# xcompact3d/x3d2

Hardware: AMD Instinct MI355X
Metric: DoF*steps/s (whole node), TGV 512^3 per GPU, full fractional step (higher is better)
Workload: dtype f64; 1 GPU; TGV 512x512x512 all-periodic, Re=1600, dt=1e-3, RK3 (3 substeps/step), compact6/classic schemes, rocFFT Poisson (configs[2]); per_gpu=512^3, driver=fused, parallelism=domain decomposition 1x1x1, decomposition=yslabs, decomposition_requested=auto, poisson_z_first=228

## Files before the change

### x3d2_amd/csrc/fft512.hip

```cpp
#include "fft_util.h"

#include "fft512_core.h"
#include "spectral000.h"

struct Spec000 {
    const real_t *waves;
    SpecAB t;
    int nx, ny, nz;
    const real_t *rwT;
};

template <int MODE, int NP, bool ZH = false>
__global__ void __launch_bounds__(64 * NP, 16 / NP)
    k_fft512(real2_t *c, const real2_t *__restrict__ twg, long stride_axis, long stride_other, int nxs, Spec000 sp,
             real2_t *xbuf, int ys, int ysc)
{
    extern __shared__ real2_t tile[];
    real2_t *__restrict__ tws = tile + NP * FP;
    if (threadIdx.x < 256) tws[threadIdx.x] = twg[threadIdx.x];
    const int tid = threadIdx.x, l = tid & 63, w = __builtin_amdgcn_readfirstlane(tid >> 6);
    const int i0 = blockIdx.x * NP, m = tid & (NP - 1), r = tid / NP;
    const long base = (long)blockIdx.y * stride_other + i0;
    const bool valid = i0 + m < nxs;
    auto xaddr = [&](int t) {
        const int ch = t / ys, tt = t - ch * ys, pt = tt / ysc, t3 = tt - pt * ysc;
        return ((((long)ch * (ys / ysc) + pt) * gridDim.y + blockIdx.y) * ysc + t3) * nxs + i0 + m;
    };
    real_t rw8[8];
    if (MODE == 2 && valid && !sp.rwT) {
#pragma unroll
        for (int it = 0; it < 8; it++) {
            const real_t wv = sp.waves[((size_t)(it * 64 + r) * sp.ny + blockIdx.y) * nxs + i0 + m];
            rw8[it] = wv < 1.e-16 ? 0.0 : -1.0 / wv;
        }
    }
#pragma unroll
    for (int it = 0; it < 8; it++) {
        const int z = it * 64 + r;
        const real2_t *__restrict__ src = (MODE == 1 && xbuf) ? xbuf + xaddr(z) : c + base + (long)z * stride_axis + m;
        tile[m * FP + z] = valid ? *src : make_real2(0.0, 0.0);
    }
    __syncthreads();
    real2_t *__restrict__ pen = tile + w * FP;
    real2_t a[8];
#pragma unroll
    for (int k = 0; k < 8; k++) a[k] = pen[l + 64 * k];
    if (MODE == 1) fft512_wave<1>(a, pen, tws, l);
    else fft512_wave<-1>(a, pen, tws, l);
    if (MODE == 2 && sp.rwT) {
        const int i = i0 + w, j = blockIdx.y;
        if (i < nxs) {
            const real_t a_o = ZH ? sp.t.az[j] : sp.t.ay[j], b_o = ZH ? sp.t.bz[j] : sp.t.by[j];
            const bool f_o = ZH ? false : (j + 1) > sp.ny / 2 + 1;
            const real_t axi = sp.t.ax[i], bxi = sp.t.bx[i];
            const bool fx = ZH && (i + 1) > sp.nx / 2 + 1;
            const real_t *__restrict__ a_ax = ZH ? sp.t.ay : sp.t.az, *__restrict__ b_ax = ZH ? sp.t.by : sp.t.bz;
            const int n_ax = ZH ? sp.ny : sp.nz;
            const real_t rn = 1.0 / sp.nx / sp.ny / sp.nz;
            const real_t *__restrict__ rwp = sp.rwT + ((size_t)j * nxs + i) * 512;
#pragma unroll
            for (int kk = 0; kk < 8; kk++) {
                const int k = l + 64 * kk;
                real_t div_r = a[kk].x * rn, div_c = a[kk].y * rn;
                const real_t a_k = a_ax[k], b_k = b_ax[k];
                const bool f_k = (k + 1) > n_ax / 2 + 1;
                const Spec000Mode md = ZH ? Spec000Mode{a_o, b_o, a_k, b_k, axi, bxi, f_o, f_k, fx}
                                         : Spec000Mode{a_k, b_k, a_o, b_o, axi, bxi, f_k, f_o, fx};
                spec000_forward(div_r, div_c, md);
                const real_t rw = rwp[k];
                div_r = div_r * rw; div_c = div_c * rw;
                spec000_backward(div_r, div_c, md);
                a[kk] = make_real2(div_r, div_c);
            }
        }
        fft512_wave<1>(a, pen, tws, l);
    } else if (MODE == 2) {
#pragma unroll
        for (int k = 0; k < 8; k++) pen[l + 64 * k] = a[k];
        __syncthreads();
        const int j = blockIdx.y, i = i0 + m;
        if (valid) {
            const real_t ayj = sp.t.ay[j], byj = sp.t.by[j], axi = sp.t.ax[i], bxi = sp.t.bx[i];
            const real_t rn = 1.0 / sp.nx / sp.ny / sp.nz;
            const bool fy = (j + 1) > sp.ny / 2 + 1;
#pragma unroll
            for (int it = 0; it < 8; it++) {
                const int k = it * 64 + r;
                real2_t v = tile[m * FP + k];
                real_t div_r = v.x * rn, div_c = v.y * rn;
                const Spec000Mode md{sp.t.az[k], sp.t.bz[k], ayj, byj, axi, bxi, (k + 1) > sp.nz / 2 + 1, fy, false};
                spec000_forward(div_r, div_c, md);
                const real_t rw = rw8[it];
                div_r = div_r * rw; div_c = div_c * rw;
                spec000_backward(div_r, div_c, md);
                tile[m * FP + k] = make_real2(div_r, div_c);
            }
        }
        __syncthreads();
#pragma unroll
        for (int k = 0; k < 8; k++) a[k] = pen[l + 64 * k];
        __syncthreads();
        fft512_wave<1>(a, pen, tws, l);
    }
#pragma unroll
    for (int k = 0; k < 8; k++) pen[l + 64 * k] = a[k];
    __syncthreads();
    if (valid) {
#pragma unroll
        for (int it = 0; it < 8; it++) {
            const int z = it * 64 + r;
            real2_t *__restrict__ dstp = (MODE == 0 && xbuf) ? xbuf + xaddr(z) : c + base + (long)z * stride_axis + m;
            *dstp = tile[m * FP + z];
        }
    }
}

template <int S, int N>
__device__ __forceinline__ void dft_small(real2_t (&v)[8])
{
    if constexpr (N == 8) fft8<S>(v);
    else if constexpr (N == 4) {
        const real2_t c0 = cadd(v[0], v[2]), c1 = cadd(v[1], v[3]), c2 = csub(v[0], v[2]), d = csub(v[1], v[3]);
        const real2_t c3 = make_real2(-S * d.y, S * d.x);
        v[0] = cadd(c0, c1); v[2] = csub(c0, c1); v[1] = cadd(c2, c3); v[3] = csub(c2, c3);
    } else if constexpr (N == 2) {
        const real2_t t0 = cadd(v[0], v[1]), t1 = csub(v[0], v[1]);
        v[0] = t0; v[1] = t1;
    }
}

struct SpecSlab {
    const real_t *waves;
    SpecAB t;
    int nx, ny, nz, nxs, yoff;
    int xoff;
// ... 112 lines not shown
template <int S, int N>
__global__ void __launch_bounds__(256) k_radix_peers(real2_t *R, long W)
{
    const long w = (long)blockIdx.x * 256 + threadIdx.x;
    const int zl = blockIdx.y;
    if (w >= W) return;
    real2_t v[8];
#pragma unroll
    for (int p = 0; p < N; p++) v[p] = R[((long)p * 512 + zl) * W + w];
    if (S < 0) dft_small<-1, N>(v);
#pragma unroll
    for (int k1 = 1; k1 < N; k1++) {
        x3d_f64 sn, cs;
        sincospi(S * 2.0 * (x3d_f64)(zl * k1) / (512.0 * N), &sn, &cs);
        v[k1] = cmul(v[k1], make_real2((real_t)cs, (real_t)sn));
    }
    if (S > 0) dft_small<1, N>(v);
#pragma unroll
    for (int p = 0; p < N; p++) R[((long)p * 512 + zl) * W + w] = v[p];
}

static real2_t *g_tw = nullptr;

template <int MODE, int NP>
static int launch512(x3d_backend *b, real2_t *c, long stride_axis, long stride_other, int nxs, int nother,
                     const Spec000 &sp, real2_t *xbuf, int ys, int ysc)
{
    const int lds = sizeof(real2_t) * (NP * FP + 256);
    X3D_LDS_OPTIN(b, (k_fft512<MODE, NP>));
    dim3 grid((nxs + NP - 1) / NP, nother);
    hipLaunchKernelGGL((k_fft512<MODE, NP>), grid, dim3(64 * NP), lds, b->stream, c, g_tw, stride_axis,
                       stride_other, nxs, sp, xbuf, ys, ysc);
    X3D_HIP(hipGetLastError());
    return 0;
}

int x3d_fft512_run_zh(x3d_backend *b, real2_t *c, long px, int kz0, int nkz, const real_t *rwZ, const real_t *ab, int nx,
                      int ny, int nz)
{
    X3D_REQUIRE(g_tw && nx == 512 && ny == 512 && nz == 512 && rwZ, "x3d_fft512_run_zh: 512^3 only");
    c += (long)kz0 * ny * px;
    SpecAB t = spec_ab_view(ab, nx, ny, nz);
    t.az += kz0; t.bz += kz0;
    const Spec000 sp{nullptr, t, nx, ny, nz, rwZ + (size_t)kz0 * 512 * 512};
    ProfScope ps(b, X3D_K_SPECTRAL, 1);
    const int lds = sizeof(real2_t) * (8 * FP + 256);
    X3D_LDS_OPTIN(b, (k_fft512<2, 8, true>));
    hipLaunchKernelGGL((k_fft512<2, 8, true>), dim3(512 / 8, nkz), dim3(512), lds, b->stream, c, g_tw, px,
                       (long)ny * px, 512, sp, nullptr, 1, 1);
    X3D_HIP(hipGetLastError());
    return 0;
}

const real2_t *x3d_fft512_twiddles() { return g_tw; }

int x3d_fft512_init()
{
    if (g_tw) return 0;
    std::vector<real2_t> h(256);
    const long double pi = 3.14159265358979323846264338327950288L;
    for (int k = 0; k < 256; k++) {
        const long double t = -2.0L * pi * k / 512.0L;
        h[k] = make_real2((real_t)cosl(t), (real_t)sinl(t));
    }
    X3D_HIP(hipMalloc(&g_tw, sizeof(real2_t) * 256));
    X3D_HIP(hipMemcpy(g_tw, h.data(), sizeof(real2_t) * 256, hipMemcpyHostToDevice));
    return 0;
}

static const real_t *g_rwT = nullptr;
void x3d_fft512_set_rwT(const real_t *rwT) { g_rwT = rwT; }

int x3d_fft512_run(x3d_backend *b, real2_t *c, int nxs, int ny, int nz, int axis, int mode, const real_t *waves,
                   const real_t *ab, int nx)
{
    return x3d_fft512_run_x(b, c, nxs, ny, nz, axis, mode, waves, ab, nx, nullptr, 1, 1);
}

int x3d_fft512_run_x(x3d_backend *b, real2_t *c, int nxs, int ny, int nz, int axis, int mode, const real_t *waves,
                     const real_t *ab, int nx, real2_t *xbuf, int ys, int ysc)
{
    const long sy = nxs, sz = (long)nxs * ny;
    const long stride_axis = axis == 1 ? sy : sz, stride_other = axis == 1 ? sz : sy;
    const int nother = axis == 1 ? nz : ny;
    X3D_REQUIRE((axis == 1 ? ny : nz) == 512, "x3d_fft512_run: axis length must be 512");
    X3D_REQUIRE(mode != 2 || axis == 2, "x3d_fft512_run: the fused pass is the z pass");
    X3D_REQUIRE(!xbuf || (axis == 1 && mode != 2 && ys > 0 && 512 % ys == 0 && ysc > 0 && ys % ysc == 0),
                "x3d_fft512_run: bad slab exchange");
    Spec000 sp{};
    if (mode == 2) sp = Spec000{waves, spec_ab_view(ab, nx, ny, nz), nx, ny, nz, g_rwT};
    const bool w16 = axis == 1;
    ProfScope ps(b, mode == 2 ? X3D_K_SPECTRAL : X3D_K_FFT, axis);
#define GO(M_, NP_) launch512<M_, NP_>(b, c, stride_axis, stride_other, nxs, nother, sp, xbuf, ys, ysc)
    if (mode == 0) return w16 ? GO(0, 16) : GO(0, 8);
    if (mode == 1) return w16 ? GO(1, 16) : GO(1, 8);
    return GO(2, 8);
#undef GO
}

__global__ void __launch_bounds__(512)
    k_r2c512(real2_t *__restrict__ c, const real_t *__restrict__ f, const real2_t *__restrict__ twg, long npairs,
             long frow, long crow)
{
    extern __shared__ real2_t tile[];
    real2_t *__restrict__ tws = tile + 8 * FP;
    if (threadIdx.x < 256) tws[threadIdx.x] = twg[threadIdx.x];
    __syncthreads();
    const int l = threadIdx.x & 63, w = __builtin_amdgcn_readfirstlane(threadIdx.x >> 6);
    real2_t *__restrict__ pen = tile + w * FP;
    for (long pr = (long)blockIdx.x * 8 + w; pr < npairs; pr += (long)gridDim.x * 8) {
        const real_t *__restrict__ fa = f + 2 * pr * frow, *__restrict__ fb = fa + frow;
        real2_t a[8];
#pragma unroll
        for (int k = 0; k < 8; k++) a[k] = make_real2(fa[l + 64 * k], fb[l + 64 * k]);
        fft512_wave<-1>(a, pen, tws, l);
#pragma unroll
// ... 94 lines not shown
```

### x3d2_amd/csrc/fft512_core.h

```cpp
#pragma once
#include "common.h"

#define FP 584

__device__ __forceinline__ real2_t cmul(real2_t a, real2_t b)
{
    return make_real2(a.x * b.x - a.y * b.y, a.x * b.y + a.y * b.x);
}
__device__ __forceinline__ real2_t cadd(real2_t a, real2_t b) { return make_real2(a.x + b.x, a.y + b.y); }
__device__ __forceinline__ real2_t csub(real2_t a, real2_t b) { return make_real2(a.x - b.x, a.y - b.y); }

template <int S>
__device__ __forceinline__ void fft8(real2_t (&a)[8])
{
    const real_t h = 0.70710678118654752440;
    real2_t b[8];
#pragma unroll
    for (int k = 0; k < 4; k++) {
        b[k] = cadd(a[k], a[k + 4]);
        b[k + 4] = csub(a[k], a[k + 4]);
    }
    {
        real2_t t = b[5];
        b[5] = make_real2(h * (t.x - S * t.y), h * (t.y + S * t.x));
        t = b[6];
        b[6] = make_real2(-S * t.y, S * t.x);
        t = b[7];
        b[7] = make_real2(h * (-t.x - S * t.y), h * (-t.y + S * t.x));
    }
#pragma unroll
    for (int o = 0; o < 8; o += 4) {
        const real2_t c0 = cadd(b[o], b[o + 2]), c1 = cadd(b[o + 1], b[o + 3]), c2 = csub(b[o], b[o + 2]);
        const real2_t d = csub(b[o + 1], b[o + 3]);
        const real2_t c3 = make_real2(-S * d.y, S * d.x);
        const int r = o ? 1 : 0;
        a[r] = cadd(c0, c1);
        a[r + 4] = csub(c0, c1);
        a[r + 2] = cadd(c2, c3);
        a[r + 6] = csub(c2, c3);
    }
}

template <int S>
__device__ __forceinline__ real2_t twiddle(const real2_t *__restrict__ tw, int e)
{
    real2_t w = tw[e & 255];
    const real_t sg = (e & 256) ? -1.0 : 1.0;
    return make_real2(sg * w.x, (S > 0 ? -sg : sg) * w.y);
}

template <int S>
__device__ __forceinline__ void fft512_wave(real2_t (&a)[8], real2_t *__restrict__ pen,
                                            const real2_t *__restrict__ tw, int l)
{
    wave_lds_fence();
    fft8<S>(a);
#pragma unroll
    for (int k1 = 1; k1 < 8; k1++) {
        a[k1] = cmul(a[k1], twiddle<S>(tw, l * k1));
    }
#pragma unroll
    for (int k1 = 0; k1 < 8; k1++) pen[k1 * 72 + l] = a[k1];
    wave_lds_fence();
    {
        const int k1 = l >> 3, b = l & 7;
#pragma unroll
        for (int q = 0; q < 8; q++) a[q] = pen[k1 * 72 + b + 8 * q];
        fft8<S>(a);
#pragma unroll
        for (int q1 = 1; q1 < 8; q1++) {
            a[q1] = cmul(a[q1], twiddle<S>(tw, 8 * b * q1));
        }
#pragma unroll
        for (int q1 = 0; q1 < 8; q1++) pen[(k1 * 8 + q1) * 9 + b] = a[q1];
    }
    wave_lds_fence();
    {
        const int k1 = l & 7, q1 = l >> 3;
#pragma unroll
        for (int b = 0; b < 8; b++) a[b] = pen[(k1 * 8 + q1) * 9 + b];
        fft8<S>(a);
    }
    wave_lds_fence();
}


#define FP256 288

template <int S>
__device__ __forceinline__ void fft4(real2_t (&a)[4])
{
    const real2_t b0 = cadd(a[0], a[2]), b1 = csub(a[0], a[2]), b2 = cadd(a[1], a[3]), d = csub(a[1], a[3]);
    const real2_t b3 = make_real2(-S * d.y, S * d.x);
    a[0] = cadd(b0, b2);
    a[2] = csub(b0, b2);
    a[1] = cadd(b1, b3);
    a[3] = csub(b1, b3);
}

template <int S>
__device__ __forceinline__ void fft256_wave(real2_t (&a)[4], real2_t *__restrict__ pen, const real2_t *__restrict__ tw,
                                            int l)
{
    wave_lds_fence();
    fft4<S>(a);
// ... 39 lines not shown
```

### x3d2_amd/csrc/xscan.hip

```cpp
#include "common.h"


int npmax_of(const x3d_backend *b);

#include "xscan_core.h"
#include "zfft_tile.h"


template <bool ACC>
__device__ __forceinline__ void store_rows_q8(real_t *__restrict__ orow, int lane, const real_t (&r)[8],
                                              real_t scale)
{
    const int j = lane & 3;
    real_t a0 = r[0], a1 = r[1], b0 = r[2], b1 = r[3], c0 = r[4], c1 = r[5], d0 = r[6], d1 = r[7];
    rotl_pairs(a0, a1, b0, b1, c0, c1, d0, d1, j);
    b0 = dpp_quad(b0, 1); b1 = dpp_quad(b1, 1);
    c0 = dpp_quad(c0, 2); c1 = dpp_quad(c1, 2);
    d0 = dpp_quad(d0, 3); d1 = dpp_quad(d1, 3);
    rotl_pairs(a0, a1, b0, b1, c0, c1, d0, d1, j);
    real2_t *__restrict__ o2 = reinterpret_cast<real2_t *>(orow + (lane & ~3) * 8) + j;
    real2_t v0, v1, v2, v3;
    if (ACC) {
        v0 = o2[0]; v1 = o2[4]; v2 = o2[8]; v3 = o2[12];
        v0.x += scale * a0; v0.y += scale * a1;
// ... 966 lines not shown
                __syncthreads();
#pragma unroll
                for (int i = 0; i < NI; i++) {
                    real2_t v = make_real2(tile[(2 * cc) * TP + cy + RP * i], tile[(2 * cc + 1) * TP + cy + RP * i]);
                    if (ACC) { v.x += old[i].x; v.y += old[i].y; }
                    {
                        real_t *q_ = reinterpret_cast<real_t *>(const_cast<real2_t *>(tile_row<RP>(o, prow, i, voff)));
                        __builtin_nontemporal_store(v.x, q_);
                        __builtin_nontemporal_store(v.y, q_ + 1);
                    }
                }
                }
            }
            __syncthreads();
        }
        if (HALO && threadIdx.x < 288) {
            const int hw = threadIdx.x / 18, k = threadIdx.x % 18;
            const long pp = (long)(tl / ntx) * (ntx * 16) + (long)(tl % ntx) * 16 + hw;
            th.bsend[((long)(k & 1) * th.nb + (k >> 1)) * th.np + pp] = bnd[threadIdx.x];
        }
    }
}

template <int Q, int MODE, bool NARROW, bool HALO, bool ZF = false, bool UNI = false, bool CIRC = false, bool CDUAL = false>
__global__ void __launch_bounds__(1024)
    k_ytile_tds_pair(real_t *out1, real_t *out2, const real_t *__restrict__ in1, const real_t *__restrict__ in2,
                     XOp ta, XOp tb, int ntx, int tile0, int ntiles, long prow, long pplane, TileHalo th, int permn,
                     ZfArg zf, CircOp ca, CircOp cb)
{
    extern __shared__ real_t lt[];
    constexpr int LN = (ZF ? LT_NC(Q) : LT_N(Q)) * 64, n = 64 * Q, TP = n + 4, NI = n / 128;
    static_assert(!ZF || (Q == 8 && MODE != 2 && !HALO), "the z-transforming forms: local pairs on 512-row pencils");
    static_assert(!CIRC || UNI, "CIRC: uniform grids");
    if constexpr (!CIRC) {
        for (int i = threadIdx.x; i < LN; i += blockDim.x) {
            lt[i] = ta.TL[i];
            if (MODE != 2) lt[LN + i] = tb.TL[i];
        }
    }
    const real_t *__restrict__ la = lt, *__restrict__ lb = lt + LN;
    real_t *tile = lt + (CIRC ? 0 : (MODE == 2 ? 1 : 2) * LN);
    real2_t *tws = reinterpret_cast<real2_t *>(tile + ZF_AREA_DOUBLES);
    if (ZF && threadIdx.x < 256) tws[threadIdx.x] = zf.tw[threadIdx.x];
    const long kzs = (long)zf.ny * zf.px;
    auto zf_row = [&](int tl) {
        int r = tl / ntx;
        if (zf.permn > 0 && r < zf.permn) r = (r & 1) ? zf.permn - ((r + 1) >> 1) : (r >> 1);
        return zf.c + (long)r * zf.px + (long)(tl % ntx) * 16;
    };
    constexpr bool NOPREF = HALO && MODE == 0;
    real_t *hal = tile + 16 * TP, *bnd = hal + 128;
    ntiles += tile0;
    int lane = threadIdx.x & 63;
// ... 130 lines not shown
            }
        }
        if constexpr (CIRC && CDUAL && MODE != 2) {
            V2 w2[Q + 8], X2[Q];
            if (MODE == 0) {
#pragma unroll
                for (int m = 0; m < Q + 8; m++) w2[m].a = w[m];
                to_tile(g2);
                __syncthreads();
                pick(b);
                window_from_body<Q>(w, b, lane);
#pragma unroll
                for (int m = 0; m < Q + 8; m++) w2[m].b = w[m];
            } else {
#pragma unroll
                for (int m = 0; m < Q + 8; m++) w2[m] = V2{w[m], w[m]};
            }
            circ_solve<Q, NARROW, V2, CircOp2>(w2, X2, circ_pair(ca, cb), lane);
            if (MODE == 0) {
#pragma unroll
                for (int q = 0; q < Q; q++) ra[q] = X2[q].a + 1.0 * X2[q].b;
                put(ra);
                __syncthreads();
                if constexpr (ZF) zf_forward<TP>(tile, tws, zf_row(tl), kzs, wave, lane);
                else from_tile(out1 + tile_off_p(tl));
            } else {
#pragma unroll
                for (int q = 0; q < Q; q++) { ra[q] = X2[q].a; rb[q] = X2[q].b; }
                put(ra);
                __syncthreads();
                from_tile(out1 + off);
                __syncthreads();
                put(rb);
                __syncthreads();
                from_tile(out2 + off);
            }
        } else {
        solve(w, ra, la, ta, 0);
        if (MODE == 0) {
            to_tile(g2);
            if (HALO && threadIdx.x < 128) hal[threadIdx.x] = h2;
            __syncthreads();
            pick(b);
            if constexpr (HALO) window_from_body_halo<Q>(w, b, lane, hal + wave * 8);
            else window_from_body<Q>(w, b, lane);
            asm volatile("" : "+v"(lane) : "v"(ra[0]));
            solve(w, rb, lb, tb, 1);
#pragma unroll
            for (int q = 0; q < Q; q++) ra[q] = ra[q] + 1.0 * rb[q];
            put(ra);
            __syncthreads();
            if constexpr (ZF) zf_forward<TP>(tile, tws, zf_row(tl), kzs, wave, lane);
            else from_tile(out1 + tile_off_p(tl));
        } else if (MODE == 1) {
            put(ra);
            __syncthreads();
            from_tile(out1 + off);
            asm volatile("" : "+v"(lane) : "v"(ra[0]));
            solve(w, rb, lb, tb, 1);
            __syncthreads();
            put(rb);
            __syncthreads();
            from_tile(out2 + off);
        } else {
            put(ra);
            __syncthreads();
            from_tile(out1 + off);
        }
        }
        if (HALO && threadIdx.x < 64) {
            const int hw = threadIdx.x >> 2, k = threadIdx.x & 3;
            const long pp = (long)(tl / ntx) * (ntx * 16) + (long)(tl % ntx) * 16 + hw;
            if ((k >> 1) < th.nb) th.bsend[((long)(k & 1) * th.nb + (k >> 1)) * th.np + pp] = bnd[threadIdx.x];
        }
        __syncthreads();
// ... 368 lines not shown
#undef GOM
#undef GON
#undef GOH
#undef GO
    if (halo) b->n_halo++;
    X3D_HIP(hipGetLastError());
    *done = true;
    return 0;
}

bool x3d_zfirst_pairs_ok(const x3d_backend *b, const x3d_tdsops *ta, const x3d_tdsops *tb)
{
    if (!use_ytile() || !xscan_ok(ta) || !xscan_ok(tb) || ta->tab.Q != 8 || tb->tab.Q != 8) return false;
    auto fast = [&](const x3d_tdsops *t) { return t->tab.bulk_only && t->n_tds == 512 && t->tab.n_rhs == t->n_tds; };
    if (!fast(ta) || !fast(tb) || b->nz != 512 || b->nx % 16 != 0) return false;
    if (sizeof(real_t) * ((size_t)2 * LT_NC(8) * 64 + ZF_AREA_DOUBLES + 512) > 160 * 1024) return false;
    return 128 * (long)b->nxp * b->nyp * X3D_RB < (1L << 32);
}

int x3d_ytile_tds_pair_zf(x3d_backend *b, int mode, real_t *out1, real_t *out2, const real_t *in1, const real_t *in2,
                          const x3d_tdsops *ta, const x3d_tdsops *tb, const ZfArg &zf, bool *done, int y0, int nyr)
{
    *done = false;
    if (mode < 0 || mode > 1 || zf.ny > b->ny || (zf.permn == 0 && zf.ny != b->ny) || !x3d_zfirst_pairs_ok(b, ta, tb)) return 0;
    if (nyr < 0) { y0 = 0; nyr = zf.ny; }
    X3D_REQUIRE(y0 >= 0 && nyr >= 0 && y0 + nyr <= zf.ny, "tds_pair (z-first): rows [%d, %d) of %d", y0, y0 + nyr, zf.ny);
    X3D_REQUIRE(zf.permn == 0 || (zf.permn == zf.ny && y0 == 0 && nyr == zf.ny), "tds_pair (z-first): interleaved rows, whole blocks only");
    if (nyr == 0) { *done = true; return 0; }
    const bool narrow = stencil_narrow(ta) && stencil_narrow(tb);
    static int uni_on = -1;
    if (uni_on < 0) { const char *e = getenv("X3D_NO_UNIFORM"); uni_on = (e && e[0] == '1') ? 0 : 1; }
    const bool uni = uni_on && ta->uniform && tb->uniform;
    const bool circ = narrow && uni && circ_env_on() && ta->circ_ok && tb->circ_ok;
    const size_t lds = sizeof(real_t) * ((size_t)(circ ? 0 : 2 * LT_NC(8) * 64) + ZF_AREA_DOUBLES + 512);
    const long pxy = (long)b->nxp * b->nyp;
    const int ntx = b->nx / 16, ntiles = ntx * nyr, tile0 = ntx * y0;
    const int blocks = x3d_persistent_blocks(b, ntiles);
    const TileHalo th{nullptr, nullptr, 0, 0, 0, 0, 0};
    ProfScope ps(b, X3D_K_TDS_FWD, X3D_DIR_Z);
#define GOD(M_, N_, U_, C_, D_)                                                                                 \
    do {                                                                                                        \
        X3D_LDS_OPTIN(b, (k_ytile_tds_pair<8, M_, N_, false, true, U_, C_, D_>));                               \
        hipLaunchKernelGGL((k_ytile_tds_pair<8, M_, N_, false, true, U_, C_, D_>), dim3(blocks), dim3(1024), lds, b->stream, out1, \
                           out2, in1, in2, xop_of(ta), xop_of(tb), ntx, tile0, ntiles, pxy, (long)b->nxp, th, 0, zf, ta->circ, tb->circ); \
    } while (0)
#define GO(M_, N_, U_, C_) GOD(M_, N_, U_, C_, (C_) && (M_) == 1)
#define GOU(M_) do { if (circ) GO(M_, true, true, true); else if (narrow && uni) GO(M_, true, true, false); else if (narrow) GO(M_, true, false, false); else GO(M_, false, false, false); } while (0)
    if (mode == 0) GOU(0); else GOU(1);
#undef GOU
#undef GO
#undef GOD
    X3D_HIP(hipGetLastError());
    *done = true;
    return 0;
}

int x3d_tds_halo_fix(x3d_backend *b, int dir, int mode, real_t *out1, real_t *out2, const real_t *brecv,
                     const x3d_tdsops *ta, const x3d_tdsops *tb)
{
    const PencilGeom g = x3d_geom(b, dir);
    const bool hc = pair_halo_circ(b, dir, ta, mode == 2 ? ta : tb);
    const TdsTab &tta = hc ? ta->tabc : ta->tab, &ttb = hc ? tb->tabc : tb->tab;
    const int wsa = hc ? ta->halo_ws_c : ta->halo_ws, wsb = hc ? tb->halo_ws_c : tb->halo_ws;
    const int wea = hc ? ta->halo_we_c : ta->halo_we, web = hc ? tb->halo_we_c : tb->halo_we;
    const int ws = mode == 2 ? wsa : (wsa > wsb ? wsa : wsb);
    const int we = mode == 2 ? wea : (wea > web ? wea : web);
    dim3 grid((g.np + 255) / 256, ws + we >= ta->n_tds ? 1 : 2);
    const int ws1 = grid.y == 1 ? ta->n_tds : ws;
    const int permn = b->pair_yperm;
    X3D_REQUIRE(permn == 0 || (dir == X3D_DIR_Z && mode != 2), "tds_halo_fix: interleaved rows are for z pairs");
    ProfScope ps(b, X3D_K_TDS_BWD, dir);
    if (mode == 0) hipLaunchKernelGGL(k_tds_halo_fix<0>, grid, dim3(256), 0, b->stream, out1, out2, brecv, tta, ttb, g, ws1, we, permn);
    else if (mode == 1) hipLaunchKernelGGL(k_tds_halo_fix<1>, grid, dim3(256), 0, b->stream, out1, out2, brecv, tta, ttb, g, ws1, we, permn);
    else hipLaunchKernelGGL(k_tds_halo_fix<2>, grid, dim3(256), 0, b->stream, out1, out2, brecv, tta, tta, g, ws1, we, 0);
// ... 249 lines not shown
```

### x3d2_amd/csrc/zfft_tile.h

```cpp
#pragma once
#include "fft512_core.h"

#define ZF_AREA_DOUBLES 9216
#define ZF_PEN 576

struct ZfArg {
    real2_t *c;
    const real2_t *tw;
    int ny;
    long px;
    int permn;
};

__device__ __forceinline__ int zf_t2(int m, int x) { return m * 16 + (x ^ (m & 15)); }

template <int TP>
__device__ __forceinline__ void zf_forward(real_t *__restrict__ area, const real2_t *__restrict__ tws,
                                           real2_t *__restrict__ crow, long kzstride, int wave, int lane)
{
    real2_t a[8], A[5], B[5];
    real2_t *__restrict__ T2 = reinterpret_cast<real2_t *>(area);
    if (wave < 8) {
        const real_t *__restrict__ pa = area + (2 * wave) * TP, *__restrict__ pb = pa + TP;
#pragma unroll
        for (int k = 0; k < 8; k++) a[k] = make_real2(pa[lane + 64 * k], pb[lane + 64 * k]);
    }
    __syncthreads();
    if (wave < 8) {
        real2_t *__restrict__ pen = T2 + wave * ZF_PEN;
        fft512_wave<-1>(a, pen, tws, lane);
#pragma unroll
        for (int k = 0; k < 8; k++) pen[lane + 64 * k] = a[k];
        wave_lds_fence();
#pragma unroll
        for (int k = 0; k < 5; k++) {
            const int idx = lane + 64 * k;
            if (k < 4 || lane == 0) {
                const real2_t x = a[k], y = pen[(512 - idx) & 511];
                A[k] = make_real2(0.5 * (x.x + y.x), 0.5 * (x.y - y.y));
                B[k] = make_real2(0.5 * (x.y + y.y), -0.5 * (x.x - y.x));
            }
        }
    }
    __syncthreads();
    if (wave < 8) {
#pragma unroll
        for (int k = 0; k < 5; k++) {
            const int idx = lane + 64 * k;
            if (k < 4 || lane == 0) {
                T2[zf_t2(idx, 2 * wave)] = A[k];
                T2[zf_t2(idx, 2 * wave + 1)] = B[k];
            }
        }
    }
    __syncthreads();
    const int r = threadIdx.x >> 4, x = threadIdx.x & 15;
#pragma unroll
    for (int i = 0; i < 5; i++) {
        const int m = r + 64 * i;
        if (i < 4 || threadIdx.x < 16) crow[(long)m * kzstride + x] = T2[zf_t2(m, x)];
    }
    __syncthreads();
}


struct ZfRows { real2_t v0, v1, v2, v3, v4; };
__device__ __forceinline__ ZfRows zf_inverse_load(const real2_t *__restrict__ crow, long kzstride)
{
    const int r = threadIdx.x >> 4, x = threadIdx.x & 15;
    const real2_t *__restrict__ p = crow + (long)r * kzstride + x;
    ZfRows v;
    v.v0 = p[0]; v.v1 = p[64 * kzstride]; v.v2 = p[128 * kzstride]; v.v3 = p[192 * kzstride];
    v.v4 = p[threadIdx.x < 16 ? 256 * kzstride : 0];
    return v;
}

template <int TP>
__device__ __forceinline__ void zf_inverse(real_t *__restrict__ area, const real2_t *__restrict__ tws,
                                           const ZfRows &v, int wave, int lane)
{
    real2_t *__restrict__ T2 = reinterpret_cast<real2_t *>(area);
    const int r = threadIdx.x >> 4, x = threadIdx.x & 15;
    T2[zf_t2(r, x)] = v.v0;
    T2[zf_t2(r + 64, x)] = v.v1;
    T2[zf_t2(r + 128, x)] = v.v2;
// ... 27 lines not shown
```

### x3d2_amd/csrc/zfirst.hip

```cpp
#include <vector>

#include "fft_util.h"
#include "poisson_priv.h"
#include "zfft_tile.h"

#define ZH_PX 520

int x3d_ztile_fft_run(x3d_backend *b, real_t *f, const ZfArg &zf, bool fwd, int y0, int nyr);

__global__ void __launch_bounds__(256)
    k_zh_rw(real_t *__restrict__ rwZ, const real_t *__restrict__ waves, int nx, int ny, int nxs)
{
    __shared__ real_t t[32][33];
    const int kz = blockIdx.z, x0 = blockIdx.x * 32, y0 = blockIdx.y * 32;
    const int tx = threadIdx.x & 31, ty = threadIdx.x >> 5;
    for (int r = ty; r < 32; r += 8) {
        const int x = x0 + tx, y = y0 + r, xm = x <= nx / 2 ? x : nx - x;
        const real_t wv = waves[((size_t)kz * ny + y) * nxs + xm];
        t[r][tx] = wv < 1.e-16 ? 0.0 : -1.0 / wv;
    }
    __syncthreads();
    for (int r = ty; r < 32; r += 8) rwZ[((size_t)kz * nx + x0 + r) * ny + y0 + tx] = t[tx][r];
}

// ... 44 lines not shown
        const real2_t t = tw1024[l + 64 * m];
        wt[m] = make_real2(t.x, S > 0 ? -t.y : t.y);
    }
    const long step = (long)gridDim.x * 8;
    for (long row = (long)blockIdx.x * 8 + w; row < nrows; row += step) {
        real2_t *__restrict__ r = c + row * pitch;
        real2_t a[8], o[8];
#pragma unroll
        for (int m = 0; m < 8; m++) {
            const real2_t lo = r[l + 64 * m], hi = r[l + 64 * (m + 8)];
            a[m] = cadd(lo, hi);
            o[m] = cmul(csub(lo, hi), wt[m]);
        }
        fft512_wave<S>(a, pen, tws, l);
        fft512_wave<S>(o, pen, tws, l);
#pragma unroll
        for (int k = 0; k < 8; k++) {
            r[2 * (l + 64 * k)] = a[k];
            r[2 * (l + 64 * k) + 1] = o[k];
        }
    }
}

template <bool FWD>
__global__ void __launch_bounds__(1024)
    k_ztile_fft(real_t *__restrict__ f, ZfArg zf, int ntx, int tile0, int ntiles, long prow, long pplane)
{
    ntiles += tile0;
    extern __shared__ real_t zarea[];
    constexpr int TP = 516;
    real2_t *__restrict__ tws = reinterpret_cast<real2_t *>(zarea + ZF_AREA_DOUBLES);
    if (threadIdx.x < 256) tws[threadIdx.x] = zf.tw[threadIdx.x];
    const int lane = threadIdx.x & 63, wave = __builtin_amdgcn_readfirstlane(threadIdx.x >> 6);
    const int cy = threadIdx.x >> 3, cc = threadIdx.x & 7;
    const long kzs = (long)zf.ny * zf.px;
    __syncthreads();
    ZfRows v{};
    if (!FWD && tile0 + (int)blockIdx.x < ntiles)
        v = zf_inverse_load(zf.c + (long)((tile0 + blockIdx.x) / ntx) * zf.px + ((tile0 + blockIdx.x) % ntx) * 16, kzs);
    for (int tl = tile0 + blockIdx.x; tl < ntiles; tl += gridDim.x) {
        const long off = (long)(tl / ntx) * pplane + (long)(tl % ntx) * 16;
        real2_t *__restrict__ crow = zf.c + (long)(tl / ntx) * zf.px + (tl % ntx) * 16;
        if (FWD) {
#pragma unroll
            for (int i = 0; i < 4; i++) {
                const real2_t g = *reinterpret_cast<const real2_t *>(f + off + (long)(cy + 128 * i) * prow + 2 * cc);
                zarea[(2 * cc) * TP + cy + 128 * i] = g.x;
                zarea[(2 * cc + 1) * TP + cy + 128 * i] = g.y;
            }
            __syncthreads();
            zf_forward<TP>(zarea, tws, crow, kzs, wave, lane);
        } else {
            zf_inverse<TP>(zarea, tws, v, wave, lane);
            const int tn = tl + gridDim.x;
            if (tn < ntiles) v = zf_inverse_load(zf.c + (long)(tn / ntx) * zf.px + (tn % ntx) * 16, kzs);
#pragma unroll
            for (int i = 0; i < 4; i++)
                *reinterpret_cast<real2_t *>(f + off + (long)(cy + 128 * i) * prow + 2 * cc) =
                    make_real2(zarea[(2 * cc) * TP + cy + 128 * i], zarea[(2 * cc + 1) * TP + cy + 128 * i]);
            __syncthreads();
        }
    }
}

static bool zfirst_sizes(const x3d_poisson *p)
{
    const x3d_backend *b = p->b;
    return p->fast512 && p->nx == 512 && p->ny == 512 && p->nz == 512 && b->nx == 512 && b->ny == 512 && b->nz == 512 &&
           (size_t)257 * 512 * ZH_PX <= (size_t)p->nz * p->ny * p->nxs && !p->stretched;
}

#define ZH010_PX 1040
int x3d_y010_run(x3d_backend *b, real2_t *c, int nxs, int nx, int ny, int nz, int mode, const real_t *tables, int sym,
                 real_t *const lu[2], bool *done, int nzl);
// ... 144 lines not shown
    p->ext_middle = middle; p->ext_user = user;
    p->ext_c = reinterpret_cast<real2_t *>(spectrum); p->ext_ny = ny; p->ext_px = px;
    if (int rc = x3d_fft512_init()) return rc;
    *out = p;
    return 0;
}
int x3d_proxy_hook(x3d_poisson *p, int which, real_t *f)
{
    if (which == 1) return p->ext_middle(p->ext_user);
    ZfArg zf{p->ext_c, x3d_fft512_twiddles(), p->ext_ny, p->ext_px, 0};
    return x3d_ztile_fft_run(p->b, f, zf, which == 0, 0, -1);
}

int x3d_ztile_fft_run(x3d_backend *b, real_t *f, const ZfArg &zf, bool fwd, int y0, int nyr)
{
    X3D_REQUIRE(b->nz == 512 && b->nx % 16 == 0 && zf.ny <= b->ny && zf.permn == 0, "x3d_ztile_fft_run: 512-row z pencils");
    if (nyr < 0) { y0 = 0; nyr = zf.ny; }
    X3D_REQUIRE(y0 >= 0 && y0 + nyr <= zf.ny, "x3d_ztile_fft_run: rows [%d, %d) of %d", y0, y0 + nyr, zf.ny);
    if (nyr == 0) return 0;
    const int ntx = b->nx / 16, ntiles = ntx * nyr, tile0 = ntx * y0;
    const size_t lds = sizeof(real_t) * (ZF_AREA_DOUBLES + 512);
    const long pxy = (long)b->nxp * b->nyp;
    ProfScope ps(b, X3D_K_FFT, 3);
    if (fwd) {
        X3D_LDS_OPTIN(b, (k_ztile_fft<true>));
        hipLaunchKernelGGL((k_ztile_fft<true>), dim3(ntiles < 512 ? ntiles : 512), dim3(1024), lds, b->stream, f, zf, ntx, tile0, ntiles, pxy, (long)b->nxp);
    } else {
        X3D_LDS_OPTIN(b, (k_ztile_fft<false>));
        hipLaunchKernelGGL((k_ztile_fft<false>), dim3(ntiles < 512 ? ntiles : 512), dim3(1024), lds, b->stream, f, zf, ntx, tile0, ntiles, pxy, (long)b->nxp);
    }
    X3D_HIP(hipGetLastError());
    return 0;
}

static int ztile(x3d_poisson *p, real_t *f, bool fwd)
{
    ZfArg zf;
    bool ok = false;
    if (int rc = x3d_zfirst_arg(p, &zf, &ok)) return rc;
    X3D_REQUIRE(ok && !p->stretched, "x3d_poisson_zfirst: not a 512^3 all-periodic solver (x3d_poisson_zfirst_ok)");
    return x3d_ztile_fft_run(p->b, f, zf, fwd, 0, -1);
}

extern "C" int x3d_poisson_zfirst_forward(x3d_poisson *p, const real_t *f_in)
{
    X3D_RANGE(__func__);
    X3D_REQUIRE(p && f_in, "x3d_poisson_zfirst_forward: null argument");
// ... 34 lines not shown
```

Before: 3.419 billion DoF*steps/s.

## Run first/last FFT512 radix-8 passes in registers and restructure z-first real split

The 512-point FFT kernel now applies the first radix-8 pass directly on the globally loaded values in registers and the last pass on registers before the store, so one full LDS round trip per pencil is skipped on load and on store. The padded row pitch changes to 577, and pass_b/pass_c take configurable strides. The z-first forward real-to-complex split is rewritten to write pencils to LDS and form the even/odd spectra in one gather; the old path stays behind an env flag. cmul and fft8 are also reshaped to use FMAs. The risks are extra register pressure and different LDS bank-conflict patterns.

```diff
diff --git a/x3d2_amd/csrc/fft512.hip b/x3d2_amd/csrc/fft512.hip
--- a/x3d2_amd/csrc/fft512.hip
+++ b/x3d2_amd/csrc/fft512.hip
@@ -10,13 +10,15 @@
     const real_t *rwT;
 };
 
-template <int MODE, int NP, bool ZH = false>
+#define FPR 577
+
+template <int MODE, int NP, bool ZH = false, bool ROWS = true>
 __global__ void __launch_bounds__(64 * NP, 16 / NP)
     k_fft512(real2_t *c, const real2_t *__restrict__ twg, long stride_axis, long stride_other, int nxs, Spec000 sp,
              real2_t *xbuf, int ys, int ysc)
 {
     extern __shared__ real2_t tile[];
-    real2_t *__restrict__ tws = tile + NP * FP;
+    real2_t *__restrict__ tws = tile + NP * FPR;
     if (threadIdx.x < 256) tws[threadIdx.x] = twg[threadIdx.x];
     const int tid = threadIdx.x, l = tid & 63, w = __builtin_amdgcn_readfirstlane(tid >> 6);
     const int i0 = blockIdx.x * NP, m = tid & (NP - 1), r = tid / NP;
@@ -34,19 +36,52 @@
             rw8[it] = wv < 1.e-16 ? 0.0 : -1.0 / wv;
         }
     }
-#pragma unroll
-    for (int it = 0; it < 8; it++) {
-        const int z = it * 64 + r;
-        const real2_t *__restrict__ src = (MODE == 1 && xbuf) ? xbuf + xaddr(z) : c + base + (long)z * stride_axis + m;
-        tile[m * FP + z] = valid ? *src : make_real2(0.0, 0.0);
-    }
-    __syncthreads();
-    real2_t *__restrict__ pen = tile + w * FP;
+    real2_t *__restrict__ pen = tile + w * FPR;
     real2_t a[8];
-#pragma unroll
-    for (int k = 0; k < 8; k++) a[k] = pen[l + 64 * k];
-    if (MODE == 1) fft512_wave<1>(a, pen, tws, l);
-    else fft512_wave<-1>(a, pen, tws, l);
+    constexpr int S0 = MODE == 1 ? 1 : -1;
+    if constexpr (ROWS) {
+#pragma unroll
+        for (int it = 0; it < 8; it++) {
+            const int z = it * 64 + r;
+            const real2_t *__restrict__ src = (MODE == 1 && xbuf) ? xbuf + xaddr(z) : c + base + (long)z * stride_axis + m;
+            a[it] = valid ? *src : make_real2(0.0, 0.0);
+        }
+        fft512_pass_a<S0>(a, twg, r);
+#pragma unroll
+        for (int k1 = 0; k1 < 8; k1++) tile[m * FPR + k1 * 72 + r] = a[k1];
+        __syncthreads();
+        if constexpr (MODE == 2) {
+            fft512_pass_b<S0, 65, 8>(a, pen, tws, l);
+            wave_lds_fence();
+            fft512_pass_c<S0, 65, 8>(a, pen, l);
+            wave_lds_fence();
+        }
+    } else {
+#pragma unroll
+        for (int it = 0; it < 8; it++) {
+            const int z = it * 64 + r;
+            const real2_t *__restrict__ src = (MODE == 1 && xbuf) ? xbuf + xaddr(z) : c + base + (long)z * stride_axis + m;
+            tile[m * FPR + z] = valid ? *src : make_real2(0.0, 0.0);
+        }
+        __syncthreads();
+#pragma unroll
+        for (int k = 0; k < 8; k++) a[k] = pen[l + 64 * k];
+        fft512_wave<S0>(a, pen, tws, l);
+    }
+    auto last_wave = [&]() {
+        if constexpr (ROWS) {
+            if constexpr (MODE == 2) {
+                wave_lds_fence();
+                fft512_pass_a<1>(a, tws, l);
+#pragma unroll
+                for (int k1 = 0; k1 < 8; k1++) pen[k1 * 72 + l] = a[k1];
+                wave_lds_fence();
+            }
+            fft512_pass_b<(MODE == 0 ? -1 : 1)>(a, pen, tws, l);
+        } else if constexpr (MODE == 2) {
+            fft512_wave<1>(a, pen, tws, l);
+        }
+    };
     if (MODE == 2 && sp.rwT) {
         const int i = i0 + w, j = blockIdx.y;
         if (i < nxs) {
@@ -73,7 +108,7 @@
                 a[kk] = make_real2(div_r, div_c);
             }
         }
-        fft512_wave<1>(a, pen, tws, l);
+        last_wave();
     } else if (MODE == 2) {
 #pragma unroll
         for (int k = 0; k < 8; k++) pen[l + 64 * k] = a[k];
@@ -86,31 +121,40 @@
 #pragma unroll
             for (int it = 0; it < 8; it++) {
                 const int k = it * 64 + r;
-                real2_t v = tile[m * FP + k];
+                real2_t v = tile[m * FPR + k];
                 real_t div_r = v.x * rn, div_c = v.y * rn;
                 const Spec000Mode md{sp.t.az[k], sp.t.bz[k], ayj, byj, axi, bxi, (k + 1) > sp.nz / 2 + 1, fy, false};
                 spec000_forward(div_r, div_c, md);
                 const real_t rw = rw8[it];
                 div_r = div_r * rw; div_c = div_c * rw;
                 spec000_backward(div_r, div_c, md);
-                tile[m * FP + k] = make_real2(div_r, div_c);
+                tile[m * FPR + k] = make_real2(div_r, div_c);
             }
         }
         __syncthreads();
 #pragma unroll
         for (int k = 0; k < 8; k++) a[k] = pen[l + 64 * k];
         __syncthreads();
-        fft512_wave<1>(a, pen, tws, l);
-    }
-#pragma unroll
-    for (int k = 0; k < 8; k++) pen[l + 64 * k] = a[k];
-    __syncthreads();
+        last_wave();
+    } else {
+        last_wave();
+    }
+    if constexpr (ROWS) {
+        __syncthreads();
+        fft512_pass_c<(MODE == 0 ? -1 : 1)>(a, tile + m * FPR, r);
+    } else {
+#pragma unroll
+        for (int k = 0; k < 8; k++) pen[l + 64 * k] = a[k];
+        __syncthreads();
+#pragma unroll
+        for (int it = 0; it < 8; it++) a[it] = tile[m * FPR + it * 64 + r];
+    }
     if (valid) {
 #pragma unroll
         for (int it = 0; it < 8; it++) {
             const int z = it * 64 + r;
             real2_t *__restrict__ dstp = (MODE == 0 && xbuf) ? xbuf + xaddr(z) : c + base + (long)z * stride_axis + m;
-            *dstp = tile[m * FP + z];
+            *dstp = a[it];
         }
     }
 }
@@ -269,14 +313,21 @@
 
 static real2_t *g_tw = nullptr;
 
-template <int MODE, int NP>
+static bool fft512_rows()
+{
+    static int rows = -1;
+    if (rows < 0) { const char *e = getenv("X3D_FFT512_NO_ROWS"); rows = !(e && e[0] == '1'); }
+    return rows;
+}
+
+template <int MODE, int NP, bool ROWS>
 static int launch512(x3d_backend *b, real2_t *c, long stride_axis, long stride_other, int nxs, int nother,
                      const Spec000 &sp, real2_t *xbuf, int ys, int ysc)
 {
-    const int lds = sizeof(real2_t) * (NP * FP + 256);
-    X3D_LDS_OPTIN(b, (k_fft512<MODE, NP>));
+    const int lds = sizeof(real2_t) * (NP * FPR + 256);
+    X3D_LDS_OPTIN(b, (k_fft512<MODE, NP, false, ROWS>));
     dim3 grid((nxs + NP - 1) / NP, nother);
-    hipLaunchKernelGGL((k_fft512<MODE, NP>), grid, dim3(64 * NP), lds, b->stream, c, g_tw, stride_axis,
+    hipLaunchKernelGGL((k_fft512<MODE, NP, false, ROWS>), grid, dim3(64 * NP), lds, b->stream, c, g_tw, stride_axis,
                        stride_other, nxs, sp, xbuf, ys, ysc);
     X3D_HIP(hipGetLastError());
     return 0;
@@ -291,10 +342,16 @@
     t.az += kz0; t.bz += kz0;
     const Spec000 sp{nullptr, t, nx, ny, nz, rwZ + (size_t)kz0 * 512 * 512};
     ProfScope ps(b, X3D_K_SPECTRAL, 1);
-    const int lds = sizeof(real2_t) * (8 * FP + 256);
-    X3D_LDS_OPTIN(b, (k_fft512<2, 8, true>));
-    hipLaunchKernelGGL((k_fft512<2, 8, true>), dim3(512 / 8, nkz), dim3(512), lds, b->stream, c, g_tw, px,
-                       (long)ny * px, 512, sp, nullptr, 1, 1);
+    const int lds = sizeof(real2_t) * (8 * FPR + 256);
+    if (fft512_rows()) {
+        X3D_LDS_OPTIN(b, (k_fft512<2, 8, true, true>));
+        hipLaunchKernelGGL((k_fft512<2, 8, true, true>), dim3(512 / 8, nkz), dim3(512), lds, b->stream, c, g_tw, px,
+                           (long)ny * px, 512, sp, nullptr, 1, 1);
+    } else {
+        X3D_LDS_OPTIN(b, (k_fft512<2, 8, true, false>));
+        hipLaunchKernelGGL((k_fft512<2, 8, true, false>), dim3(512 / 8, nkz), dim3(512), lds, b->stream, c, g_tw, px,
+                           (long)ny * px, 512, sp, nullptr, 1, 1);
+    }
     X3D_HIP(hipGetLastError());
     return 0;
 }
@@ -338,7 +395,9 @@
     if (mode == 2) sp = Spec000{waves, spec_ab_view(ab, nx, ny, nz), nx, ny, nz, g_rwT};
     const bool w16 = axis == 1;
     ProfScope ps(b, mode == 2 ? X3D_K_SPECTRAL : X3D_K_FFT, axis);
-#define GO(M_, NP_) launch512<M_, NP_>(b, c, stride_axis, stride_other, nxs, nother, sp, xbuf, ys, ysc)
+#define GO(M_, NP_)                                                                                          \
+    (fft512_rows() ? launch512<M_, NP_, true>(b, c, stride_axis, stride_other, nxs, nother, sp, xbuf, ys, ysc) \
+                   : launch512<M_, NP_, false>(b, c, stride_axis, stride_other, nxs, nother, sp, xbuf, ys, ysc))
     if (mode == 0) return w16 ? GO(0, 16) : GO(0, 8);
     if (mode == 1) return w16 ? GO(1, 16) : GO(1, 8);
     return GO(2, 8);
diff --git a/x3d2_amd/csrc/fft512_core.h b/x3d2_amd/csrc/fft512_core.h
--- a/x3d2_amd/csrc/fft512_core.h
+++ b/x3d2_amd/csrc/fft512_core.h
@@ -5,7 +5,7 @@
 
 __device__ __forceinline__ real2_t cmul(real2_t a, real2_t b)
 {
-    return make_real2(a.x * b.x - a.y * b.y, a.x * b.y + a.y * b.x);
+    return make_real2(fma_r(a.x, b.x, -(a.y * b.y)), fma_r(a.x, b.y, a.y * b.x));
 }
 __device__ __forceinline__ real2_t cadd(real2_t a, real2_t b) { return make_real2(a.x + b.x, a.y + b.y); }
 __device__ __forceinline__ real2_t csub(real2_t a, real2_t b) { return make_real2(a.x - b.x, a.y - b.y); }
@@ -20,18 +20,21 @@
         b[k] = cadd(a[k], a[k + 4]);
         b[k + 4] = csub(a[k], a[k + 4]);
     }
+    real2_t c1o, d_o;
     {
         real2_t t = b[5];
-        b[5] = make_real2(h * (t.x - S * t.y), h * (t.y + S * t.x));
+        const real2_t u5 = make_real2(t.x - S * t.y, t.y + S * t.x);
         t = b[6];
         b[6] = make_real2(-S * t.y, S * t.x);
         t = b[7];
-        b[7] = make_real2(h * (-t.x - S * t.y), h * (-t.y + S * t.x));
+        const real2_t b7 = make_real2(h * (-t.x - S * t.y), h * (-t.y + S * t.x));
+        c1o = make_real2(fma_r(h, u5.x, b7.x), fma_r(h, u5.y, b7.y));
+        d_o = make_real2(fma_r(h, u5.x, -b7.x), fma_r(h, u5.y, -b7.y));
     }
 #pragma unroll
     for (int o = 0; o < 8; o += 4) {
-        const real2_t c0 = cadd(b[o], b[o + 2]), c1 = cadd(b[o + 1], b[o + 3]), c2 = csub(b[o], b[o + 2]);
-        const real2_t d = csub(b[o + 1], b[o + 3]);
+        const real2_t c0 = cadd(b[o], b[o + 2]), c1 = o ? c1o : cadd(b[1], b[3]), c2 = csub(b[o], b[o + 2]);
+        const real2_t d = o ? d_o : csub(b[1], b[3]);
         const real2_t c3 = make_real2(-S * d.y, S * d.x);
         const int r = o ? 1 : 0;
         a[r] = cadd(c0, c1);
@@ -50,37 +53,52 @@
 }
 
 template <int S>
+__device__ __forceinline__ void fft512_pass_a(real2_t (&a)[8], const real2_t *__restrict__ tw, int p)
+{
+    fft8<S>(a);
+#pragma unroll
+    for (int k1 = 1; k1 < 8; k1++) {
+        a[k1] = cmul(a[k1], twiddle<S>(tw, p * k1));
+    }
+}
+
+template <int S, int S1 = 72, int S2 = 9>
+__device__ __forceinline__ void fft512_pass_b(real2_t (&a)[8], real2_t *__restrict__ pen, const real2_t *__restrict__ tw,
+                                              int l)
+{
+    const int k1 = l >> 3, b = l & 7;
+#pragma unroll
+    for (int q = 0; q < 8; q++) a[q] = pen[k1 * 72 + b + 8 * q];
+    fft8<S>(a);
+#pragma unroll
+    for (int q1 = 1; q1 < 8; q1++) {
+        a[q1] = cmul(a[q1], twiddle<S>(tw, 8 * b * q1));
+    }
+#pragma unroll
+    for (int q1 = 0; q1 < 8; q1++) pen[k1 * S1 + q1 * S2 + b] = a[q1];
+}
+
+template <int S, int S1 = 72, int S2 = 9>
+__device__ __forceinline__ void fft512_pass_c(real2_t (&a)[8], const real2_t *__restrict__ pen, int p)
+{
+    const int k1 = p & 7, q1 = p >> 3;
+#pragma unroll
+    for (int b = 0; b < 8; b++) a[b] = pen[k1 * S1 + q1 * S2 + b];
+    fft8<S>(a);
+}
+
+template <int S>
 __device__ __forceinline__ void fft512_wave(real2_t (&a)[8], real2_t *__restrict__ pen,
                                             const real2_t *__restrict__ tw, int l)
 {
     wave_lds_fence();
-    fft8<S>(a);
-#pragma unroll
-    for (int k1 = 1; k1 < 8; k1++) {
-        a[k1] = cmul(a[k1], twiddle<S>(tw, l * k1));
-    }
+    fft512_pass_a<S>(a, tw, l);
 #pragma unroll
     for (int k1 = 0; k1 < 8; k1++) pen[k1 * 72 + l] = a[k1];
     wave_lds_fence();
-    {
-        const int k1 = l >> 3, b = l & 7;
-#pragma unroll
-        for (int q = 0; q < 8; q++) a[q] = pen[k1 * 72 + b + 8 * q];
-        fft8<S>(a);
-#pragma unroll
-        for (int q1 = 1; q1 < 8; q1++) {
-            a[q1] = cmul(a[q1], twiddle<S>(tw, 8 * b * q1));
-        }
-#pragma unroll
-        for (int q1 = 0; q1 < 8; q1++) pen[(k1 * 8 + q1) * 9 + b] = a[q1];
-    }
+    fft512_pass_b<S>(a, pen, tw, l);
     wave_lds_fence();
-    {
-        const int k1 = l & 7, q1 = l >> 3;
-#pragma unroll
-        for (int b = 0; b < 8; b++) a[b] = pen[(k1 * 8 + q1) * 9 + b];
-        fft8<S>(a);
-    }
+    fft512_pass_c<S>(a, pen, l);
     wave_lds_fence();
 }
 
diff --git a/x3d2_amd/csrc/xscan.hip b/x3d2_amd/csrc/xscan.hip
--- a/x3d2_amd/csrc/xscan.hip
+++ b/x3d2_amd/csrc/xscan.hip
@@ -1012,13 +1012,14 @@
     }
 }
 
-template <int Q, int MODE, bool NARROW, bool HALO, bool ZF = false, bool UNI = false, bool CIRC = false, bool CDUAL = false>
+template <int Q, int MODE, bool NARROW, bool HALO, int ZFK = 0, bool UNI = false, bool CIRC = false, bool CDUAL = false>
 __global__ void __launch_bounds__(1024)
     k_ytile_tds_pair(real_t *out1, real_t *out2, const real_t *__restrict__ in1, const real_t *__restrict__ in2,
                      XOp ta, XOp tb, int ntx, int tile0, int ntiles, long prow, long pplane, TileHalo th, int permn,
                      ZfArg zf, CircOp ca, CircOp cb)
 {
     extern __shared__ real_t lt[];
+    constexpr bool ZF = ZFK != 0;
     constexpr int LN = (ZF ? LT_NC(Q) : LT_N(Q)) * 64, n = 64 * Q, TP = n + 4, NI = n / 128;
     static_assert(!ZF || (Q == 8 && MODE != 2 && !HALO), "the z-transforming forms: local pairs on 512-row pencils");
     static_assert(!CIRC || UNI, "CIRC: uniform grids");
@@ -1195,7 +1196,7 @@
                 for (int q = 0; q < Q; q++) ra[q] = X2[q].a + 1.0 * X2[q].b;
                 put(ra);
                 __syncthreads();
-                if constexpr (ZF) zf_forward<TP>(tile, tws, zf_row(tl), kzs, wave, lane);
+                if constexpr (ZF) zf_forward<TP, ZFK == 2>(tile, tws, zf_row(tl), kzs, wave, lane);
                 else from_tile(out1 + tile_off_p(tl));
             } else {
 #pragma unroll
@@ -1223,7 +1224,7 @@
             for (int q = 0; q < Q; q++) ra[q] = ra[q] + 1.0 * rb[q];
             put(ra);
             __syncthreads();
-            if constexpr (ZF) zf_forward<TP>(tile, tws, zf_row(tl), kzs, wave, lane);
+            if constexpr (ZF) zf_forward<TP, ZFK == 2>(tile, tws, zf_row(tl), kzs, wave, lane);
             else from_tile(out1 + tile_off_p(tl));
         } else if (MODE == 1) {
             put(ra);
@@ -1638,6 +1639,7 @@
                           const x3d_tdsops *ta, const x3d_tdsops *tb, const ZfArg &zf, bool *done, int y0, int nyr)
 {
     *done = false;
+    const bool split8 = zf_split8_env();
     if (mode < 0 || mode > 1 || zf.ny > b->ny || (zf.permn == 0 && zf.ny != b->ny) || !x3d_zfirst_pairs_ok(b, ta, tb)) return 0;
     if (nyr < 0) { y0 = 0; nyr = zf.ny; }
     X3D_REQUIRE(y0 >= 0 && nyr >= 0 && y0 + nyr <= zf.ny, "tds_pair (z-first): rows [%d, %d) of %d", y0, y0 + nyr, zf.ny);
@@ -1654,11 +1656,16 @@
     const int blocks = x3d_persistent_blocks(b, ntiles);
     const TileHalo th{nullptr, nullptr, 0, 0, 0, 0, 0};
     ProfScope ps(b, X3D_K_TDS_FWD, X3D_DIR_Z);
+#define GOZ(M_, N_, U_, C_, D_, Z_)                                                                             \
+    do {                                                                                                        \
+        X3D_LDS_OPTIN(b, (k_ytile_tds_pair<8, M_, N_, false, Z_, U_, C_, D_>));                                 \
+        hipLaunchKernelGGL((k_ytile_tds_pair<8, M_, N_, false, Z_, U_, C_, D_>), dim3(blocks), dim3(1024), lds, b->stream, out1, \
+                           out2, in1, in2, xop_of(ta), xop_of(tb), ntx, tile0, ntiles, pxy, (long)b->nxp, th, 0, zf, ta->circ, tb->circ); \
+    } while (0)
 #define GOD(M_, N_, U_, C_, D_)                                                                                 \
     do {                                                                                                        \
-        X3D_LDS_OPTIN(b, (k_ytile_tds_pair<8, M_, N_, false, true, U_, C_, D_>));                               \
-        hipLaunchKernelGGL((k_ytile_tds_pair<8, M_, N_, false, true, U_, C_, D_>), dim3(blocks), dim3(1024), lds, b->stream, out1, \
-                           out2, in1, in2, xop_of(ta), xop_of(tb), ntx, tile0, ntiles, pxy, (long)b->nxp, th, 0, zf, ta->circ, tb->circ); \
+        constexpr int Z2 = (M_) == 0 ? 2 : 1;                                                                   \
+        if (split8 && Z2 == 2) GOZ(M_, N_, U_, C_, D_, Z2); else GOZ(M_, N_, U_, C_, D_, 1);                    \
     } while (0)
 #define GO(M_, N_, U_, C_) GOD(M_, N_, U_, C_, (C_) && (M_) == 1)
 #define GOU(M_) do { if (circ) GO(M_, true, true, true); else if (narrow && uni) GO(M_, true, true, false); else if (narrow) GO(M_, true, false, false); else GO(M_, false, false, false); } while (0)
@@ -1666,6 +1673,7 @@
 #undef GOU
 #undef GO
 #undef GOD
+#undef GOZ
     X3D_HIP(hipGetLastError());
     *done = true;
     return 0;
diff --git a/x3d2_amd/csrc/zfft_tile.h b/x3d2_amd/csrc/zfft_tile.h
--- a/x3d2_amd/csrc/zfft_tile.h
+++ b/x3d2_amd/csrc/zfft_tile.h
@@ -14,11 +14,20 @@
 
 __device__ __forceinline__ int zf_t2(int m, int x) { return m * 16 + (x ^ (m & 15)); }
 
-template <int TP>
+static inline int zf_split8_env()
+{
+    static int v = -1;
+    if (v < 0) { const char *e = getenv("X3D_ZF_SPLIT8"); v = (e && e[0] == '1') ? 1 : 0; }
+    return v;
+}
+
+__device__ __forceinline__ int zf_z(int pair, int m) { return pair * ZF_PEN + ((m + 2 * pair) & 511); }
+
+template <int TP, bool SPLIT8 = false>
 __device__ __forceinline__ void zf_forward(real_t *__restrict__ area, const real2_t *__restrict__ tws,
                                            real2_t *__restrict__ crow, long kzstride, int wave, int lane)
 {
-    real2_t a[8], A[5], B[5];
+    real2_t a[8];
     real2_t *__restrict__ T2 = reinterpret_cast<real2_t *>(area);
     if (wave < 8) {
         const real_t *__restrict__ pa = area + (2 * wave) * TP, *__restrict__ pb = pa + TP;
@@ -26,6 +35,28 @@
         for (int k = 0; k < 8; k++) a[k] = make_real2(pa[lane + 64 * k], pb[lane + 64 * k]);
     }
     __syncthreads();
+    const int r = threadIdx.x >> 4, x = threadIdx.x & 15;
+    if constexpr (!SPLIT8) {
+        if (wave < 8) {
+            fft512_wave<-1>(a, T2 + wave * ZF_PEN, tws, lane);
+#pragma unroll
+            for (int k = 0; k < 8; k++) T2[zf_z(wave, lane + 64 * k)] = a[k];
+        }
+        __syncthreads();
+#pragma unroll
+        for (int i = 0; i < 5; i++) {
+            const int m = r + 64 * i;
+            if (i < 4 || threadIdx.x < 16) {
+                const real2_t p = T2[zf_z(x >> 1, m)], y = T2[zf_z(x >> 1, (512 - m) & 511)];
+                const bool odd = x & 1;
+                const real_t re = odd ? 0.5 * (p.y + y.y) : 0.5 * (p.x + y.x);
+                const real_t im = odd ? -0.5 * (p.x - y.x) : 0.5 * (p.y - y.y);
+                crow[(long)m * kzstride + x] = make_real2(re, im);
+            }
+        }
+        __syncthreads();
+    } else {
+    real2_t A[5], B[5];
     if (wave < 8) {
         real2_t *__restrict__ pen = T2 + wave * ZF_PEN;
         fft512_wave<-1>(a, pen, tws, lane);
@@ -36,9 +67,9 @@
         for (int k = 0; k < 5; k++) {
             const int idx = lane + 64 * k;
             if (k < 4 || lane == 0) {
-                const real2_t x = a[k], y = pen[(512 - idx) & 511];
-                A[k] = make_real2(0.5 * (x.x + y.x), 0.5 * (x.y - y.y));
-                B[k] = make_real2(0.5 * (x.y + y.y), -0.5 * (x.x - y.x));
+                const real2_t p = a[k], y = pen[(512 - idx) & 511];
+                A[k] = make_real2(0.5 * (p.x + y.x), 0.5 * (p.y - y.y));
+                B[k] = make_real2(0.5 * (p.y + y.y), -0.5 * (p.x - y.x));
             }
         }
     }
@@ -54,13 +85,13 @@
         }
     }
     __syncthreads();
-    const int r = threadIdx.x >> 4, x = threadIdx.x & 15;
 #pragma unroll
     for (int i = 0; i < 5; i++) {
         const int m = r + 64 * i;
         if (i < 4 || threadIdx.x < 16) crow[(long)m * kzstride + x] = T2[zf_t2(m, x)];
     }
     __syncthreads();
+    }
 }
 
 
diff --git a/x3d2_amd/csrc/zfirst.hip b/x3d2_amd/csrc/zfirst.hip
--- a/x3d2_amd/csrc/zfirst.hip
+++ b/x3d2_amd/csrc/zfirst.hip
@@ -90,7 +90,7 @@
     }
 }
 
-template <bool FWD>
+template <bool FWD, bool SPLIT8 = false>
 __global__ void __launch_bounds__(1024)
     k_ztile_fft(real_t *__restrict__ f, ZfArg zf, int ntx, int tile0, int ntiles, long prow, long pplane)
 {
@@ -117,7 +117,7 @@
                 zarea[(2 * cc + 1) * TP + cy + 128 * i] = g.y;
             }
             __syncthreads();
-            zf_forward<TP>(zarea, tws, crow, kzs, wave, lane);
+            zf_forward<TP, SPLIT8>(zarea, tws, crow, kzs, wave, lane);
         } else {
             zf_inverse<TP>(zarea, tws, v, wave, lane);
             const int tn = tl + gridDim.x;
@@ -308,7 +308,10 @@
     const size_t lds = sizeof(real_t) * (ZF_AREA_DOUBLES + 512);
     const long pxy = (long)b->nxp * b->nyp;
     ProfScope ps(b, X3D_K_FFT, 3);
-    if (fwd) {
+    if (fwd && zf_split8_env()) {
+        X3D_LDS_OPTIN(b, (k_ztile_fft<true, true>));
+        hipLaunchKernelGGL((k_ztile_fft<true, true>), dim3(ntiles < 512 ? ntiles : 512), dim3(1024), lds, b->stream, f, zf, ntx, tile0, ntiles, pxy, (long)b->nxp);
+    } else if (fwd) {
         X3D_LDS_OPTIN(b, (k_ztile_fft<true>));
         hipLaunchKernelGGL((k_ztile_fft<true>), dim3(ntiles < 512 ? ntiles : 512), dim3(1024), lds, b->stream, f, zf, ntx, tile0, ntiles, pxy, (long)b->nxp);
     } else {
```

After: 3.358 billion DoF*steps/s. 0.982x the previous value.
